# Astropianist/LumFuncMCMC

Hardware: AMD Instinct MI355X
Metric: walker-lnprob evals/sec (10^6 sources, 256 walkers) (higher is better)
Workload: dtype f64; 1 GPU; free completeness, single Schechter: 1000000 synthetic sources, 256 walkers in all (256 per GPU), 2 half-ensemble calls of 128 theta rows per step; walkers_per_gpu=256, walkers_total=256, variant=free, parallelism=1 GPU

## Files before the change

lumfuncmcmc_amd/csrc/lf_free.h:

```cpp
#pragma once
#include "lf_tile.h"

namespace lf {


template <bool THROUGH = false>
__device__ __forceinline__ void reduce_store512(const double* __restrict__ red, int wlo, int whi, double* __restrict__ out,
                                                size_t stride, int w0, int chunk, int tid) {
    const int w = tid >> 6, lane = tid & 63;
    if (w >= wlo && w < whi) {
        const double* row = red + w * PB + lane;
        double s0 = (row[0] + row[64]) + (row[128] + row[192]);
        double s1 = (row[256] + row[320]) + (row[384] + row[448]);
        const double s = wave_sum_dpp(s0 + s1);
        if (lane == 63) {
            if (THROUGH) __hip_atomic_store(out + (size_t)(w0 + w) * stride + chunk, s, __ATOMIC_RELAXED, __HIP_MEMORY_SCOPE_AGENT);
            else out[(size_t)(w0 + w) * stride + chunk] = s;
        }
    }
}

struct FreeArgs {
    int B, ntiles;
    int nchA, nchB;
    int nslot;
    int tile_stride;
    int skip_grid;
    int* queues;
    double* partA;
    double* partB;
    const double* cells;
    const double* nodes8;
    const int* deal;
    const int* cc_len;
    const int* cc_field;
    int nchC;
    int fin_ranks;
    double* partC;
    const int* wstat;
    const double* theta;
    double* out;
    double* wrec_w;
    int* wmode_w;
    int* wstat_w;
    double* wbase_w;
    const double* gq_rec;
    const double* gq_omega;
    const int* gq_rows;
    int nbq;
    int poll;
    int* err;
};

template <int ST, bool CENSUS, bool FUSED, bool STEP, class LA>
__device__ __forceinline__ void lf_free_body(const KConst& kc, const SrcArrays& sa, const NodeArrays& na, const double* __restrict__ wrec_arg,
                                             const int* __restrict__ wmode_arg, const FreeArgs& fa, const LA& la, const StepArgs& sp,
                                             const AcceptArgs& ap, unsigned long long t_pre = 0) {
    const double* wrec = FUSED ? fa.wrec_w : wrec_arg;
    const int* wmode = FUSED ? fa.wmode_w : wmode_arg;
    __shared__ MathTables tab;
    __shared__ TermTables tt;
    __shared__ __attribute__((aligned(16))) double red[PTW * PB];
    __shared__ __attribute__((aligned(16))) double wfc[PTW * MAXF * 8];
    __shared__ __attribute__((aligned(16))) double wsc[PTW * 8];
    __shared__ int sitem[2];
    __shared__ int sdeal[DEAL_MAX];
    __shared__ int scell;
    __shared__ int snosrc;
    const int tid = threadIdx.x;
    __shared__ int sstat[PTW];
    __shared__ double sbase[PTW];
    __shared__ double wlf[PTW * MAXF];
    __shared__ double sprop[PTW * 16];
    __shared__ double szz[PTW];
    __shared__ double spre[PTW * 2];
    if (!FUSED) {
        for (int i = tid; i < 256; i += PB) {
            tab.logt[i] = *reinterpret_cast<const double2*>(LOG_TABLE + 2 * i);
            tab.expt[i] = EXP_TABLE[i];
        }
        load_term_tables<PB>(&tt);
        if (fa.deal && tid < DEAL_LIST + fa.nchC + fa.nbq) sdeal[tid] = fa.deal[tid];
    }
    bool tables_loaded = !FUSED;
    const int wave_base = __builtin_amdgcn_readfirstlane(tid & ~63);
    auto fresh_tid = [&]() -> int {
        int m = -1;
        asm volatile("" : "+s"(m));
        return wave_base + __builtin_amdgcn_mbcnt_hi(m, __builtin_amdgcn_mbcnt_lo(m, 0));
    };
    unsigned xcc;
    asm volatile("s_getreg_b32 %0, hwreg(HW_REG_XCC_ID)" : "=s"(xcc));
    const int myq = (int)(xcc & 7u);
#ifdef LF_STAMPS
    __shared__ unsigned long long s_targs;
    unsigned long long* stamp = kc.stamps ? kc.stamps + (size_t)blockIdx.x * 8 : nullptr;
    if (stamp && tid == 0) {
        stamp[0] = t_pre ? t_pre : __builtin_amdgcn_s_memtime();
        stamp[5] = __builtin_amdgcn_s_memrealtime();
        s_targs = __builtin_amdgcn_s_memtime();
    }
    int nitems_done = 0;
    unsigned long long t_first = 0, t_sw = 0, t_loop = 0, t_red = 0;
    unsigned long long t_prep = 0, t_cells = 0, t_grid = 0;
    __shared__ unsigned long long s_ttab;
    __shared__ unsigned long long s_tp0;
    __shared__ unsigned long long s_tprep[8];
#endif

#pragma unroll 1
    for (int tile = ((int)blockIdx.x >> 3) % la.ntiles; tile < la.ntiles; tile += la.tile_stride) {
        const int w0 = tile * PTW;
        const int nw = min(PTW, la.B - w0);
        __builtin_assume(nw >= 1 && nw <= PTW);
        int* __restrict__ q = fa.queues + tile * QSTRIDE;
        int fgroup, frank;
        tile_ranks(tile, la.ntiles, la.tile_stride, fgroup, frank);
        const bool finisher = FUSED && fa.poll && frank == tile_finisher(fa.fin_ranks, fgroup);
        bool no_src = false;
        auto grab = [&]() -> int {
            if (no_src) return -1;
            for (int d = 0; d < 8; ++d) {
                const int qq = (myq + d) & 7;
                const int lo = (int)(((long long)qq * fa.nchA) >> 3), hi = (int)(((long long)(qq + 1) * fa.nchA) >> 3);
                if (hi <= lo) continue;
                const int i = atomicAdd(q + 1 + qq, 1);
                if (i < hi - lo) return lo + i;
            }
            return -1;
        };
        int ticket = 0;
        auto take_ticket = [&]() {
            if (!no_src) ticket = atomicAdd(q + 1 + myq, 1);
        };
        auto redeem = [&]() -> int {
            if (no_src) return -1;
            const int lo = (int)(((long long)myq * fa.nchA) >> 3), hi = (int)(((long long)(myq + 1) * fa.nchA) >> 3);
            if (ticket < hi - lo) return lo + ticket;
            return grab();
        };
        if (tile != ((int)blockIdx.x >> 3) % la.ntiles) __syncthreads();
        const int u = fresh_tid();
        if (FUSED) {
            const int pw = (int)(blockIdx.x >> 8) & 1;
            const int up = u - 64 * pw;
            if (up >= 0 && up < 64) {
                prepare_lane<false, true, STEP, LF_FREE>(kc, sp, la.theta, la.B, nullptr, nullptr, nullptr, nullptr, nullptr, 1,
                                          w0 + (up >> 3), up & 7, up >> 3, reinterpret_cast<double(*)[16]>(red), wfc, wsc, sstat, sbase, wlf,
#ifdef LF_STAMPS
                                          s_tprep,
#else
                                          nullptr,
#endif
                                          sprop, szz);
#ifdef LF_STAMPS
                if (up == 0) s_tp0 = __builtin_amdgcn_s_memtime();
#endif
            } else if (!tables_loaded) {
                const int t7 = u < 64 * pw ? u : u - 64;
                double2 lt = *reinterpret_cast<const double2*>(LOG_TABLE + 2 * min(t7, 255));
                double et = EXP_TABLE[min(t7, 255)];
                const int ndeal = fa.deal ? DEAL_LIST + fa.nchC + fa.nbq : 0;
                int d0 = ndeal ? fa.deal[min(t7, ndeal - 1)] : 0, d1 = ndeal ? fa.deal[min(t7 + 256, ndeal - 1)] : 0;
                asm volatile("" : "+v"(lt.x), "+v"(lt.y), "+v"(et), "+v"(d0), "+v"(d1));
                load_term_tables<PB - 64>(&tt, t7);
                if (t7 < 256) {
                    tab.logt[t7] = lt;
                    tab.expt[t7] = et;
                    if (t7 < ndeal) sdeal[t7] = d0;
                    if (t7 + 256 < ndeal) sdeal[t7 + 256] = d1;
                }
#ifdef LF_STAMPS
                if (t7 == 0) s_ttab = __builtin_amdgcn_s_memtime();
#endif
            }
            accept_terms_ahead<STEP>(sp, ap, w0, nw, u, spre);
            tables_loaded = true;
            __syncthreads();
        }
        if (u < 64) {
            const int st = FUSED ? sstat[min(u, nw - 1)] : fa.wstat[w0 + min(u, nw - 1)];
            const bool on = fa.nchC > 0 && u < nw && (st & STAT_CELLS);
            const bool need = u < nw && !on && (st & STAT_PRIOR_OK) && !(st & STAT_NEGINF);
            const int m = (int)__ballot(on);
            const unsigned long long mneed = __ballot(need);
            if (u == 0) {
                scell = m;
                no_src = mneed == 0ull;
                snosrc = no_src ? 1 : 0;
                sitem[0] = grab();
            }
        }
        if (!FUSED && u < nw * MAXF) {
            const int w = u / MAXF, f = u - w * MAXF;
            double* d = wfc + u * 8;
            int* di = reinterpret_cast<int*>(d + 4);
            if (f < kc.nf) {
                const double* __restrict__ r = wrec + (size_t)(w0 + w) * REC;
                const int* __restrict__ km = wmode + ((size_t)(w0 + w) * MAXF + f) * WM;
                d[0] = r[R_ALPHAC];
                d[F_V] = r[RF(f, F_V)];
                d[F_CA] = r[RF(f, F_CA)];
                d[F_CY] = r[RF(f, F_CY)] - H_LO - 0.5 / H_INV;
                d[7] = r[RF(f, F_CY)] - H_LO;
#pragma unroll
                for (int i = 0; i < 5; ++i) di[i] = km[i];
            }
        }
        if (!FUSED && u >= PB - PTW * 8) {
            const int t = u - (PB - PTW * 8), w = t >> 3, j = t & 7;
            if (w < nw) wsc[t] = wrec[(size_t)(w0 + w) * REC + j];
        }
        __syncthreads();
#ifdef LF_STAMPS
        t_prep = __builtin_amdgcn_s_memtime();
#endif
        const int cellmask = __builtin_amdgcn_readfirstlane(scell);
        const bool keep_own = finisher && uni(snosrc);
        double* __restrict__ sown = red + PB;
        auto fetch = [&](int w, int fld) {
            const double2* __restrict__ p = reinterpret_cast<const double2*>(wfc + (w * MAXF + fld) * 8);
            const double2 a = p[0], b = p[1], c = p[3];
            if (FUSED) {
                const int* __restrict__ ki = reinterpret_cast<const int*>(wfc + (w * MAXF + fld) * 8 + 4);
                return WalkerK{a.x, b.x, b.y, c.y, uni(ki[M_MODE]), uni(ki[M_KLO]), uni(ki[M_KHI]), uni(ki[M_KNE]), uni(ki[M_KAC])};
            }
            const int* __restrict__ km = wmode + ((size_t)(w0 + w) * MAXF + fld) * WM;
            return WalkerK{a.x, b.x, b.y, c.y, km[M_MODE], km[M_KLO], km[M_KHI], km[M_KNE], km[M_KAC]};
        };

        {
            const int v = wave_base >> 6;
#pragma unroll 1
            for (int vr = frank; vr < VF; vr += fgroup) {
            double acc = 0.0;
            const bool dealt = fa.deal != nullptr;
            const int cfirst = (vr - VF / 2 + VF) % VF;
            const int cb = dealt ? DEAL_LIST + uni(sdeal[vr]) : cfirst;
            const int cn = dealt ? uni(sdeal[vr + 1]) - uni(sdeal[vr]) : (cfirst < fa.nchC ? (fa.nchC - cfirst + VF - 1) / VF : 0);
            auto chunk_at = [&](int i) { return dealt ? uni(sdeal[cb + i]) : cb + i * VF; };
            if (fa.nchC > 0 && v < nw && ((cellmask >> v) & 1) && cn > 0) {
                auto load_cells = [&](double (&d)[CELL_REC], int cc) {
                    const int lane = fresh_tid() & 63;
                    const double2* __restrict__ src = reinterpret_cast<const double2*>(fa.cells + ((size_t)cc * 64 + lane) * CELL_REC);
                    static_assert(CELL_REC % 2 == 0, "16-byte loads");
#pragma unroll
                    for (int k = 0; k < CELL_REC / 2; ++k) {
                        const double2 a = src[k];
                        d[2 * k] = a.x;
                        d[2 * k + 1] = a.y;
                    }
                };
                auto field_of = [&](int cc) {
                    int f = 0;
#pragma unroll
                    for (int k = 1; k < MAXF; ++k) f += cc >= kc.cc_fstart[k] ? 1 : 0;
                    return f;
                };
                double nx[CELL_REC];
                load_cells(nx, chunk_at(0));
#pragma unroll 1
                for (int ci = 0; ci < cn; ++ci) {
                    const int cc = chunk_at(ci);
                    double cd[CELL_REC];
#pragma unroll
                    for (int k = 0; k < CELL_REC; ++k) cd[k] = nx[k];
                    if (ci + 1 < cn) load_cells(nx, chunk_at(ci + 1));
                    const WalkerK p = fetch(v, field_of(cc));
                    asm volatile("; LF_BEGIN cell items=1");
                    acc += cell_sum(cd, p, &tt);
                    asm volatile("; LF_END cell");
                    if (CENSUS && kc.forms && (fresh_tid() & 63) == 0) atomicAdd(kc.forms + FORM_CELL, (unsigned long long)uni(fa.cc_len[cc]));
                }
            }
            if (fa.nchC > 0 && v < nw) {
                acc = wave_sum_dpp(acc);
                const int ln = fresh_tid() & 63;
                double* __restrict__ row = fa.partC + (size_t)(w0 + v) * fa.nslot;
                if (ln == 63) {
                    if (keep_own) sown[v * 128 + vr] = acc;
                    else pstore<FUSED>(row + vr, acc);
                }
            }
            }
        }
#ifdef LF_STAMPS
        t_cells = __builtin_amdgcn_s_memtime();
#endif
        if (fa.nbq > 0) {
            const int v = wave_base >> 6;
            const int nq = fa.nbq;
#pragma unroll 1
            for (int vr = frank; vr < VF; vr += fgroup) {
            double bsum = 0.0;
            const bool dealt = fa.deal != nullptr;
            const int qb = dealt ? DEAL_LIST + fa.nchC + uni(sdeal[DEAL_BINS + vr]) : vr;
            const int qn = dealt ? uni(sdeal[DEAL_BINS + vr + 1]) - uni(sdeal[DEAL_BINS + vr]) : (vr < nq ? (nq - vr + VF - 1) / VF : 0);
            auto bin_at = [&](int i) { return dealt ? uni(sdeal[qb + i]) : qb + i * VF; };
            if (v < nw && qn > 0) {
                const double* __restrict__ sc = wsc + v * 8;
                const int mode = __builtin_amdgcn_readfirstlane(*reinterpret_cast<const int*>(wfc + (v * MAXF) * 8 + 4));
                const double* __restrict__ r = wfc + v * MAXF * 8 - 8;
                double vmin = r[RF(0, F_V)];
                for (int f = 1; f < kc.nf; ++f) vmin = fmin(vmin, r[RF(f, F_V)]);
                vmin = uni(vmin);
                const double alphaC = uni(sc[R_ALPHAC]);
                auto mine = [&](int c) { return mode != MODE_SKIP && !(kc.grid_parts > 1 && c % kc.grid_parts != kc.grid_part); };
                struct QRec {
                    double x, a4, L, PGL;
                };
                auto load_rec = [&](int c) -> QRec {
                    const int lane = fresh_tid() & 63;
                    const double2* __restrict__ src = reinterpret_cast<const double2*>(fa.gq_rec + ((size_t)c * 64 + lane) * 4);
                    const double2 a = src[0], b = src[1];
                    return QRec{a.x, a.y, b.x, b.y};
                };
                double* __restrict__ Tl = red + v * 64;
                QRec nx = load_rec(bin_at(0));
#pragma unroll 1
                for (int qi = 0; qi < qn; ++qi) {
                    const int c = bin_at(qi);
                    const QRec nd = nx;
                    const int nr = uni(fa.gq_rows[4 * c + 1]), off = uni(fa.gq_rows[4 * c + 2]);
                    if (qi + 1 < qn) nx = load_rec(bin_at(qi + 1));
                    if (mine(c)) {
                        const int lane = fresh_tid() & 63;
                        const double* __restrict__ om = fa.gq_omega + off + lane;
                        double o[8];
#pragma unroll
                        for (int i = 0; i < 8; ++i) o[i] = i < nr ? om[i * 64] : 0.0;
                        asm volatile("; LF_BEGIN qT items=1");
                        Tl[lane] = fexp_c(fma(uni(sc[R_C1]), nd.L - uni(sc[R_LSTAR]), uni(sc[R_C0])) - nd.PGL * uni(sc[R_Q]), &tab);
                        asm volatile("; LF_END qT");
                        const double a4min = __hiloint2double(__builtin_amdgcn_readlane(__double2hiint(nd.a4), 63),
                                                              __builtin_amdgcn_readlane(__double2loint(nd.a4), 63));
                        const bool bright = kc.specialise && alphaC > 0.0 && a4min * vmin > 37.5;
                        if (CENSUS && kc.forms && lane == 0)
                            atomicAdd(kc.forms + (bright ? FORM_NODE_BRIGHT : FORM_NODE_GENERAL), (unsigned long long)(64 * kc.nf));
                        const double s = field_sum_nf(kc, r, alphaC, nd.x, nd.a4, &tab, bright);
                        __builtin_amdgcn_wave_barrier();
                        asm volatile("; LF_BEGIN qdot items=1");
                        double R = 0.0;
#pragma unroll 1
                        for (int k0 = 0; k0 < nr; k0 += 8) {
                            double on[8];
#pragma unroll
                            for (int i = 0; i < 8; ++i) on[i] = k0 + 8 + i < nr ? om[(k0 + 8 + i) * 64] : 0.0;
#pragma unroll
                            for (int i = 0; i < 8; ++i) R = fma(Tl[min(k0 + i, 63)], o[i], R);
#pragma unroll
                            for (int i = 0; i < 8; ++i) o[i] = on[i];
                        }
                        asm volatile("; LF_END qdot");
                        bsum = fma(R, s, bsum);
                        __builtin_amdgcn_wave_barrier();
                    }
                }
            }
            if (v < nw) {
                bsum = wave_sum_dpp(bsum);
                const int ln = fresh_tid() & 63;
                double* __restrict__ row = fa.partB + (size_t)(w0 + v) * fa.nslot;
                if (ln == 63) {
                    if (keep_own) sown[v * 128 + 64 + vr] = bsum;
                    else pstore<FUSED>(row + vr, bsum);
                }
            }
            }
        } else
        {
            const int v = wave_base >> 6;
            const int nch64 = fa.nchB;
#pragma unroll 1
            for (int vr = frank; vr < VF; vr += fgroup) {
            double bsum = 0.0;
            if (v < nw && vr < nch64) {
                const double* __restrict__ sc = wsc + v * 8;
                const int mode = __builtin_amdgcn_readfirstlane(*reinterpret_cast<const int*>(wfc + (v * MAXF) * 8 + 4));
                const double* __restrict__ r = wfc + v * MAXF * 8 - 8;
                double vmin = r[RF(0, F_V)];
                for (int f = 1; f < kc.nf; ++f) vmin = fmin(vmin, r[RF(f, F_V)]);
                vmin = uni(vmin);
                const double alphaC = uni(sc[R_ALPHAC]);
                auto mine = [&](int c) { return mode != MODE_SKIP && !(kc.grid_parts > 1 && c % kc.grid_parts != kc.grid_part); };
                struct Node {
                    double G, PG, W, a3, a4, a4min;
                };
                auto load_nodes = [&](int c) -> Node {
                    const int lane = fresh_tid() & 63;
                    const double2* __restrict__ src = reinterpret_cast<const double2*>(fa.nodes8 + ((size_t)c * 64 + lane) * 8);
                    const double2 a = src[0], b = src[1], d = src[2];
                    return Node{a.x, a.y, b.x, b.y, d.x, d.y};
                };
                Node nx = load_nodes(vr);
#pragma unroll 1
                for (int c = vr; c < nch64; c += VF) {
                    const Node nd = nx;
                    if (c + VF < nch64) nx = load_nodes(c + VF);
                    if (mine(c)) {
                        const double a4min = uni(nd.a4min);
                        const double T = fexp_c(fma(uni(sc[R_C1]), nd.G - uni(sc[R_LSTAR]), uni(sc[R_C0])) - nd.PG * uni(sc[R_Q]), &tab);
                        const bool bright = kc.specialise && alphaC > 0.0 && a4min * vmin > 37.5;
                        if (CENSUS && kc.forms && (fresh_tid() & 63) == 0)
                            atomicAdd(kc.forms + (bright ? FORM_NODE_BRIGHT : FORM_NODE_GENERAL),
                                      (unsigned long long)(min(64, na.nnodes - c * 64) * kc.nf));
                        const double s = field_sum_nf(kc, r, alphaC, nd.a3, nd.a4, &tab, bright);
                        bsum = fma(nd.W * T, s, bsum);
                    }
                }
            }
            if (nch64 > 0 && v < nw) {
                bsum = wave_sum_dpp(bsum);
                const int ln = fresh_tid() & 63;
                double* __restrict__ row = fa.partB + (size_t)(w0 + v) * fa.nslot;
                if (ln == 63) {
                    if (keep_own) sown[v * 128 + 64 + vr] = bsum;
                    else pstore<FUSED>(row + vr, bsum);
                }
            }
            }
        }
#ifdef LF_STAMPS
        t_grid = __builtin_amdgcn_s_memtime();
#endif
        int item = sitem[0];
#pragma unroll 1
        while (item >= 0) {
#ifdef LF_STAMPS
            const unsigned long long ta = __builtin_amdgcn_s_memtime();
            if (t_first == 0) t_first = ta;
            unsigned long long tb = ta, tc = ta;
#endif
            __syncthreads();
            int t = fresh_tid();
            {
                const int c = item;
                const int s0 = uni(sa.chunk_start[c]), n = uni(sa.chunk_len[c]), fld = uni(sa.chunk_field[c]);
                const int kfirst = uni(sa.chunk_keys[KEY_STRIDE * c]), klast = uni(sa.chunk_keys[KEY_STRIDE * c + 1]),
                          kamax = uni(sa.chunk_keys[KEY_STRIDE * c + 4 + (wave_base >> 6)]);
                double x[ST];
                if (t == 0) take_ticket();
                if (n == PB * ST) {
                    typedef double __attribute__((ext_vector_type(2), aligned(8))) double2_a8;
                    const double2_a8* __restrict__ src = reinterpret_cast<const double2_a8*>(sa.a1 + s0 + t * ST);
#pragma unroll
                    for (int k = 0; k < ST / 2; ++k) {
                        const double2_a8 a = src[k];
                        x[2 * k] = a.x;
                        x[2 * k + 1] = a.y;
                    }
                } else {
                    const double* __restrict__ src = sa.a1 + s0;
#pragma unroll
                    for (int k = 0; k < ST; ++k) x[k] = src[min(t * ST + k, n - 1)];
                }
                if (t == 0) {
                    asm volatile("" ::"v"(x[ST - 1]));
                    sitem[0] = redeem();
                }
#ifdef LF_STAMPS
                tb = __builtin_amdgcn_s_memtime();
#endif
                const int npad = ST - min(max(n - t * ST, 0), ST);
                const int nwave = min(max(n - wave_base * ST, 0), 64 * ST);
                int rest = 0;
                WalkerK pn = fetch(0, fld);
#pragma unroll 1
                for (int w = 0; w < nw; ++w) {
                    const WalkerK p = pn;
                    pn = fetch(min(w + 1, nw - 1), fld);
                    double acc = 0.0;
                    if ((cellmask >> w) & 1) {
                    } else if (p.mode < MODE_SKIP && p.mode != MODE_SLOW && kc.tables && kfirst >= p.klo && klast <= p.khi && p.kac <= kamax) {
                        TabCoef C;
                        if (kc.specialise && kfirst >= p.kne) {
                            asm volatile("; LF_BEGIN table_noexp items=%0" ::"n"(ST));
                            table_lookup<ST>(C, x, p, true, &tt);
                            acc = table_terms<ST, true>(C, x, npad);
// ... 72 lines not shown
                        }
                        if (CENSUS && kc.forms && (t & 63) == 0) atomicAdd(kc.forms + form, (unsigned long long)nwave);
                        red[w * PB + t] = acc;
                    }
                }
#ifdef LF_STAMPS
                tc = __builtin_amdgcn_s_memtime();
#endif
                __syncthreads();
                t = fresh_tid();
                reduce_store512<FUSED>(red, 0, nw, fa.partA, (size_t)fa.nchA, w0, c, t);
                item = sitem[0];
            }
#ifdef LF_STAMPS
            ++nitems_done;
            if (tb != ta) {
                t_sw += tb - ta;
                t_loop += tc - tb;
                t_red += __builtin_amdgcn_s_memtime() - tc;
            }
#endif
        }
        if (FUSED && fa.poll && uni(snosrc)) {
            if (finisher) {
                const int t = fresh_tid(), v = t >> 6, ln = t & 63;
                const int nB = fa.nchB > 0 ? fa.nslot : 0, nC = fa.nchC > 0 ? fa.nslot : 0;
                if (v < nw) {
                    const bool own = ln % fgroup == frank;
                    double pre[2] = {0.0, 0.0};
                    if (own && ln < fa.nslot) pre[0] = sown[v * 128 + ln], pre[1] = sown[v * 128 + 64 + ln];
                    poll_finish(fa.partB, fa.partC, w0 + v, fa.nslot, nB, nC, ln, fa.err, pre, own);
                    finalize_wave<true>(fa.partA, 0, fa.nchA, fa.partB, nB, nB, nC > 0 ? fa.partC : nullptr, nC, (int)STAT_CELLS,
                                        sstat - w0, sbase - w0, w0 + v, ln, ap, la.out, nullptr, nullptr, 0,
                                        STEP ? sprop + v * 16 : nullptr, STEP ? szz + v : nullptr, STEP ? spre + 2 * v : nullptr, pre);
                }
            }
        } else if (FUSED) {
            count_finish(q, sitem[1], fgroup, nw, [&] { const int t = fresh_tid(); return TileThread{t, t >> 6, t & 63}; },
                         [&](int v, int ln) {
                             const int nB = fa.nchB > 0 ? fa.nslot : 0, nC = fa.nchC > 0 ? fa.nslot : 0;
                             finalize_wave<true>(fa.partA, fa.nchA, fa.nchA, fa.partB, nB, nB, nC > 0 ? fa.partC : nullptr, nC, (int)STAT_CELLS,
                                                 sstat - w0, sbase - w0, w0 + v, ln, ap, la.out, nullptr, nullptr, 0,
                                                 STEP ? sprop + v * 16 : nullptr, STEP ? szz + v : nullptr, STEP ? spre + 2 * v : nullptr);
                             if (fa.poll) empty_slots(fa.partB, fa.partC, w0 + v, fa.nslot, nB, nC, ln);
                         });
        }
    }
#ifdef LF_STAMPS
    if (stamp && tid == 0) {
        stamp[1] = __builtin_amdgcn_s_memtime();
        const bool noitems = nitems_done == 0;
        stamp[2] = (unsigned long long)nitems_done;
        if (noitems) {
            stamp[3] = t_prep - stamp[0];
            stamp[4] = t_cells - stamp[0];
            stamp[7] = t_grid - stamp[0];
            unsigned long long pk = 0;
            pk = ((s_targs - stamp[0]) >> 4) & 0xfffull;
            for (int i = 0; i < 4; ++i) pk |= (((s_tprep[i] - stamp[0]) >> 4) & 0xfffull) << (12 * (i + 1));
            stamp[2] = pk;
        } else {
            stamp[3] = t_first ? t_first - stamp[0] : 0;
            stamp[4] = t_sw;
            stamp[7] = t_loop;
        }
        stamp[6] = __builtin_amdgcn_s_memrealtime();
        kc.stamps[(size_t)gridDim.x * 8 + blockIdx.x] =
            !noitems ? t_red : (((s_ttab - stamp[0]) << 32) | ((s_tp0 - stamp[0]) & 0xffffffffull));
    }
#endif
}

template <int ST, bool CENSUS, bool FUSED = false>
__global__ __launch_bounds__(PB, 4) void lf_free(KConst kc, SrcArrays sa, NodeArrays na, const double* __restrict__ wrec_arg,
                                                 const int* __restrict__ wmode_arg, FreeArgs fa) {
    static_assert(!FUSED, "the one-launch form is the block entry below");
#ifdef LF_STAMPS
    const unsigned long long t_pre = __builtin_amdgcn_s_memtime();
#else
    const unsigned long long t_pre = 0;
#endif
    warm_kernarg<sizeof(KConst) + sizeof(SrcArrays) + sizeof(NodeArrays) + 2 * 8 + sizeof(FreeArgs)>();
    lf_free_body<ST, CENSUS, FUSED, false>(kc, sa, na, wrec_arg, wmode_arg, fa, fa, StepArgs{}, AcceptArgs{}, t_pre);
}

struct FreeLaunch {
    const double* theta;
    double* out;
    int B, ntiles;
    int tile_stride;
};
static_assert(sizeof(FreeLaunch) <= 64 - 8, "the block's pointer and the launch's fields: one line of kernel arguments");
struct FreeBlock {
    KConst kc;
    SrcArrays sa;
    NodeArrays na;
    FreeArgs fa;
};

typedef const __attribute__((address_space(4))) FreeBlock* FreeBlockPtr;

template <int ST, bool CENSUS, bool FUSED>
__global__ __launch_bounds__(PB, 4) void lf_free(FreeBlockPtr __restrict__ blkc, FreeLaunch la) {
    static_assert(FUSED && !CENSUS, "the block entry is the one-launch form");
    const FreeBlock* __restrict__ blk = (const FreeBlock*)blkc;
#ifdef LF_STAMPS
    const unsigned long long t_pre = __builtin_amdgcn_s_memtime();
// ... 15 lines not shown
```

lumfuncmcmc_amd/csrc/lf_kernels.h:

```cpp
#pragma once
#include "lf_layout.h"
#include "lf_math.h"

namespace lf {

constexpr int REC = 8 + 8 * MAXF;
constexpr int WM = 8;
enum { MODE_FAST = 0, MODE_SLOW = 1, MODE_NEGINF = 2, MODE_SKIP = 3, MODE_SKIPSRC = 4 };
enum { STAT_PRIOR_OK = 1, STAT_NEGINF = 2, STAT_SLOW = 4,
       STAT_CELLS = 8 };
constexpr int CELL_M = 8;
constexpr int CELL_REC = CELL_M + 2;
constexpr double CELL_RHO_G = 1.5e-2, CELL_RHO_H = 3.0e-3;
constexpr double ZCELL_RHO = 1.0e-3, ZCELL_X1 = 6.0e-3, ZCELL_X2 = 1.0e-5;
constexpr int ZCELL_M = 6;
constexpr int ZCELL_REC = ZCELL_M + 2;

enum { R_LSTAR = 0, R_C0 = 1, R_C1 = 2, R_Q = 3, R_ALPHAC = 4 };
enum { F_LF = 0, F_V = 1, F_CA = 2, F_CY = 3 };
__host__ __device__ constexpr int RF(int f, int slot) { return 8 + 8 * f + slot; }
enum { M_MODE = 0, M_KLO = 1, M_KHI = 2, M_KNE = 3, M_KAC = 4 };
enum { FORM_GENERAL = 0, FORM_GENERAL_NOEXP = 1, FORM_TABLE = 2, FORM_TABLE_NOEXP = 3, FORM_CAREFUL = 4, FORM_SKIPPED = 5,
       FORM_NODE_GENERAL = 6, FORM_NODE_BRIGHT = 7, FORM_CELL = 8, FORM_COUNT = 9 };
enum { Z_AL = 0, Z_BL = 1, Z_CL = 2, Z_AP = 3, Z_BP = 4, Z_CP = 5, Z_C1 = 6 };
// ... 80 lines not shown
}
__device__ __forceinline__ double u53(unsigned int hi, unsigned int lo) {
    return (double)((((unsigned long long)hi << 32) | lo) >> 11) * 1.1102230246251565e-16;
}
__device__ __forceinline__ double stretch_z(double a, double u) {
#pragma clang fp contract(off)
    const double t = (a - 1.0) * u;
    const double g = t + 1.0;
    const double g2 = g * g;
    return g2 / a;
}
__device__ __forceinline__ double stretch_point(double xj, double xk, double z) {
#pragma clang fp contract(off)
    const double d = xj - xk;
    const double dz = d * z;
    return xj - dz;
}
__device__ __forceinline__ void sampler_draw(unsigned long long step, int half, int w, int stream,
                                             unsigned long long seed, unsigned int (&r)[4]) {
    philox4x32((unsigned int)step, (unsigned int)(step >> 32) ^ ((unsigned int)half << 31), (unsigned int)w,
               (unsigned int)stream, (unsigned int)seed, (unsigned int)(seed >> 32), r);
}

template <int CTRL>
__device__ __forceinline__ int dpp_mov(int v) {
    return __builtin_amdgcn_update_dpp(0, v, CTRL, 0xf, 0xf, true);
}
template <int CTRL>
__device__ __forceinline__ double dpp_mov(double v) {
    return __hiloint2double(dpp_mov<CTRL>(__double2hiint(v)), dpp_mov<CTRL>(__double2loint(v)));
}
__device__ __forceinline__ double group8_sum(double v) {
    v += dpp_mov<0xB1>(v);
    v += dpp_mov<0x4E>(v);
    v += dpp_mov<0x141>(v);
    return v;
}
__device__ __forceinline__ int group8_or(int v) {
    v |= dpp_mov<0xB1>(v);
    v |= dpp_mov<0x4E>(v);
    v |= dpp_mov<0x141>(v);
    return v;
}

__device__ __forceinline__ int key_ceil(double v) {
    if (!(v == v)) return KEY_MAX;
    return (int)fmin(fmax(ceil(v), 0.0), (double)KEY_MAX);
}
__device__ __forceinline__ int key_floor(double v) {
    if (!(v == v)) return -1;
    return (int)fmin(fmax(floor(v), -1.0), (double)(KEY_MAX - 1));
}

template <bool BLOCK_SYNC, bool TOLDS = false, bool STEP = BLOCK_SYNC, int VAR = -1>
__device__ __forceinline__ void prepare_lane(const KConst& kc, const StepArgs& sp, const double* __restrict__ theta, int B,
                                             double* __restrict__ wrec, int* __restrict__ wstat,
                                             int* __restrict__ wmode, double* __restrict__ wbase, int* __restrict__ slow_list,
                                             int nqueue, int wq, int f, int grp, double (*sth)[16],
                                             double* __restrict__ l_fc = nullptr, double* __restrict__ l_sc = nullptr,
                                             int* __restrict__ l_stat = nullptr, double* __restrict__ l_base = nullptr,
                                             double* __restrict__ l_lf = nullptr, unsigned long long* tst = nullptr,
                                             double* __restrict__ l_prop = nullptr, double* __restrict__ l_zz = nullptr) {
#ifdef LF_STAMPS
#define LF_TST(i) do { if (tst && wq % 8 == 0 && f == 0) tst[i] = __builtin_amdgcn_s_memtime(); } while (0)
#else
#define LF_TST(i) do { } while (0)
#endif
    LF_TST(0);
    const int variant = VAR >= 0 ? VAR : kc.variant;
    const bool live = wq < B;
    const int w = live ? wq : B - 1;
    const bool has_f = f < kc.nf;
    struct {
        double pmax, lum_min, lum_max, a_min, u_min, u_max, lnom0, slc, sp, som, flim0, z_lo, z_hi, sz, sz2;
        int nsrc, kf_first, kf_last;
    } kf;
    struct {
        double lims[5][2], pivots[3], sch_al0, alpha0, fc_ratio, key_x0, zcell_rho;
    } pc;
    {
        int vz = 0;
        asm volatile("" : "+v"(vz));
        const double* __restrict__ lp = &kc.lims[0][0];
        const bool zv = variant == LF_ZEVOL;
#pragma unroll
        for (int i = 0; i < 10; ++i) pc.lims[i >> 1][i & 1] = zv && (i >> 1) >= LF_LIM_FLIM ? 0.0 : lp[i + vz];
        static_assert(LF_LIM_LSTAR < LF_LIM_FLIM && LF_LIM_PHISTAR < LF_LIM_FLIM && LF_LIM_SCH_AL < LF_LIM_FLIM && LF_LIM_ALPHA >= LF_LIM_FLIM,
                      "the z-evolving variant's limits come first");
#pragma unroll
        for (int i = 0; i < 3; ++i) pc.pivots[i] = zv ? (&kc.pivots[0])[i + vz] : 0.0;
        pc.sch_al0 = (&kc.sch_al0)[vz];
        pc.alpha0 = zv ? 0.0 : (&kc.alpha0)[vz];
        pc.fc_ratio = zv ? 0.0 : (&kc.fc_ratio)[vz];
        pc.key_x0 = zv ? 0.0 : (&kc.key_x0)[vz];
        pc.zcell_rho = zv ? (&kc.zcell_rho)[vz] : 0.0;
    }
    const bool stepping = STEP && sp.enabled;
    double t0 = 0.0, t1 = 0.0;
    if (!stepping) {
        const double* __restrict__ row = theta + (size_t)w * kc.ndim;
        t0 = row[min(f, kc.ndim - 1)];
        t1 = row[min(f + 8, kc.ndim - 1)];
    }
    kf.lum_min = kc.lum_min[f]; kf.lum_max = kc.lum_max[f]; kf.a_min = kc.a_min[f]; kf.slc = kc.slc[f]; kf.som = kc.som[f];
    kf.nsrc = kc.nsrc[f];
    if (variant == LF_ZEVOL) {
        kf.z_lo = kc.z_lo[f]; kf.z_hi = kc.z_hi[f]; kf.sz = kc.sz[f]; kf.sz2 = kc.sz2[f];
        kf.pmax = kf.u_min = kf.u_max = kf.lnom0 = kf.sp = kf.flim0 = 0.0; kf.kf_first = kf.kf_last = 0;
        asm volatile("" : "+v"(t0), "+v"(t1), "+v"(kf.lum_min), "+v"(kf.lum_max), "+v"(kf.a_min), "+v"(kf.slc), "+v"(kf.som), "+v"(kf.nsrc),
                          "+v"(kf.z_lo), "+v"(kf.z_hi), "+v"(kf.sz), "+v"(kf.sz2));
    } else {
        kf.pmax = kc.pmax[f]; kf.u_min = kc.u_min[f]; kf.u_max = kc.u_max[f]; kf.lnom0 = kc.lnom0_src[f]; kf.sp = kc.sp[f];
        kf.flim0 = kc.flim0[f]; kf.kf_first = kc.kf_first[f]; kf.kf_last = kc.kf_last[f];
        kf.z_lo = kf.z_hi = kf.sz = kf.sz2 = 0.0;
        asm volatile("" : "+v"(t0), "+v"(t1), "+v"(kf.lum_min), "+v"(kf.lum_max), "+v"(kf.a_min), "+v"(kf.slc), "+v"(kf.som), "+v"(kf.nsrc),
// ... 49 lines not shown
            const double n = (double)kf.nsrc;
            const double sph = aP * kf.sz2 + bP * kf.sz + n * cP;
            const double sls = aL * kf.sz2 + bL * kf.sz + n * (cL - LF_LREF);
            base = kf.som + n * LF_LNLN10 + LF_LN10 * sph + c1 * (kf.slc - sls);
        }
        if (live && f == 0) {
            double* d = TOLDS ? l_sc + grp * 8 : r;
            d[Z_AL] = aL; d[Z_BL] = bL; d[Z_CL] = cL;
            d[Z_AP] = aP; d[Z_BP] = bP; d[Z_CP] = cP;
            d[Z_C1] = c1;
        }
        if (live && has_f) {
            const double s0 = fabs(fma(2.0 * aL, kf.z_lo, bL)), s1 = fabs(fma(2.0 * aL, kf.z_hi, bL));
            (TOLDS ? l_fc + (grp * MAXF + f) * 8 : r + RF(f, 0))[0] = LF_LN10 * (fmax(s0, s1) + fabs(aL) * (1.0 / 128.0));
            cell_ok = kf.nsrc == 0 || (LF_LN10 * fmax(s0, s1) * pc.zcell_rho <= ZCELL_X1 &&
                                          LF_LN10 * fabs(aL) * pc.zcell_rho * pc.zcell_rho <= ZCELL_X2);
        }
        if (has_f && kf.nsrc > 0) {
            double lsmn, lsmx, phmn, phmx;
            quad_range(aL, bL, cL, kf.z_lo, kf.z_hi, lsmn, lsmx);
            quad_range(aP, bP, cP, kf.z_lo, kf.z_hi, phmn, phmx);
            const double tmax = kf.lum_max - lsmn, tmin = kf.lum_min - lsmx;
            const double vb = tmax < 2.9 ? (double)(__builtin_amdgcn_exp2f((float)tmax * 3.3219285f) * 1.0001f) + 1.0e-30 : 1.0e300;
            const double lb = LF_LNLN10 + LF_LN10 * phmn + fmin(c1 * tmin, c1 * tmax) - vb;
            m = (vb < 700.0 && lb > SAFE && lb + kf.a_min > SAFE) ? MODE_FAST : MODE_SLOW;
        }
    } else {
        const double Lstar = th[0], phistar = th[1];
        int k = 2;
        const double al = kc.fix_sch_al ? pc.sch_al0 : th[k++];
        const double alphaC = variant == LF_FREE ? th[k + kc.nf] : pc.alpha0;
        ok = ok && (Lstar >= pc.lims[LF_LIM_LSTAR][0]) && (Lstar <= pc.lims[LF_LIM_LSTAR][1]);
        ok = ok && (phistar >= pc.lims[LF_LIM_PHISTAR][0]) && (phistar <= pc.lims[LF_LIM_PHISTAR][1]);
        ok = ok && (al >= pc.lims[LF_LIM_SCH_AL][0]) && (al <= pc.lims[LF_LIM_SCH_AL][1]);
        ok = ok && (alphaC >= pc.lims[LF_LIM_ALPHA][0]) && (alphaC <= pc.lims[LF_LIM_ALPHA][1]);
        const double c0 = LF_LNLN10 + LF_LN10 * phistar, c1 = LF_LN10 * (al + 1.0);
        const double Q = exp10(LF_LREF - Lstar);
        asm volatile("" : "+v"(const_cast<double&>(Q)));
        LF_TST(2);
        if (has_f && kf.nsrc > 0) {
            const double n = (double)kf.nsrc;
            const double c0f = c0 + (variant == LF_FREE ? kf.lnom0 : 0.0);
            base = n * c0f + c1 * (kf.slc - n * (Lstar - LF_LREF)) - Q * kf.sp +
                   (variant == LF_FIXCOMP ? kf.som : 0.0);
        }
        if (live && f == 0) {
            double* d = TOLDS ? l_sc + grp * 8 : r;
            d[R_LSTAR] = Lstar;
            d[R_C0] = c0;
            d[R_C1] = c1;
            d[R_Q] = Q;
            d[R_ALPHAC] = alphaC;
        }
        if (has_f) {
            const double Flim = variant == LF_FREE ? th[k + f] : kf.flim0;
            ok = ok && (Flim >= pc.lims[LF_LIM_FLIM][0]) && (Flim <= pc.lims[LF_LIM_FLIM][1]);
            double lF = 0.0, V = 0.0;
            if (variant == LF_FREE) {
                const double b = -sqrt(pc.fc_ratio / (alphaC * alphaC));
                lF = log10(1.0e-17 * Flim);
                V = 1.0 / (Flim * exp10(b));
                const double cA = -alphaC * lF, cY = -(lF + b);
                int klo = KEY_MAX, khi = -1, kne = KEY_MAX, kac = KEY_MAX;
                if (nqueue > 0 && alphaC > 0.0 && alphaC < 1.0e4) {
                    const double xlo = fmax((G_NUM_LO + 2.0 * G_MARGIN - cA) / alphaC, H_LO + 2.0 * H_MARGIN - cY);
                    const double xhi = (G_NUM_HI - 2.0 * G_MARGIN - cA) / alphaC;
                    const double xne = 1.5740312677277188 - cY;
                    klo = key_ceil((xlo - pc.key_x0) * KEY_SCALE);
                    khi = key_floor((xhi - pc.key_x0) * KEY_SCALE);
                    kne = key_ceil((xne - pc.key_x0) * KEY_SCALE);
                    kac = key_ceil(alphaC * KEY_ASCALE);
                }
                cell_ok = kf.nsrc == 0 || (klo <= kf.kf_first && kf.kf_last <= khi);
                if (live && TOLDS) {
                    double* d = l_fc + (grp * MAXF + f) * 8;
                    int* di = reinterpret_cast<int*>(d + 4);
                    d[0] = alphaC;
                    d[F_V] = V;
                    d[F_CA] = cA;
                    d[F_CY] = cY - H_LO - 0.5 / H_INV;
                    d[7] = cY - H_LO;
                    di[M_KLO] = klo;
                    di[M_KHI] = khi;
                    di[M_KNE] = kne;
                    di[M_KAC] = kac;
                    l_lf[grp * MAXF + f] = lF;
                } else if (live) {
                    r[RF(f, F_LF)] = lF;
                    r[RF(f, F_V)] = V;
                    r[RF(f, F_CA)] = cA;
                    r[RF(f, F_CY)] = cY;
                    int* km = wmode + ((size_t)w * MAXF + f) * WM;
                    km[M_KLO] = klo;
                    km[M_KHI] = khi;
                    km[M_KNE] = kne;
                    km[M_KAC] = kac;
                }
            }
            LF_TST(3);
            if (kf.nsrc > 0) {
                const double vmax = kf.pmax * Q;
                const double tlo = kf.lum_min - Lstar, thi = kf.lum_max - Lstar;
                const double lbT = c0 + fmin(c1 * tlo, c1 * thi) - vmax;
                if (vmax > LF_UNDERFLOW) {
                    m = MODE_NEGINF;
                    neginf = 1;
                } else if (variant == LF_FREE) {
                    const double num = alphaC * (kf.a_min - lF);
                    const float an = (float)fmax(-num, 0.0);
                    const float lnfc_lo = num >= 0.0 ? -0.6932f
                                                     : -2.00002f * 0.69314724f * __builtin_amdgcn_logf(2.0f * (1.0f + an) * 1.000001f) - 0.01f;
                    const float x = (float)(kf.u_min * V) * 0.999999f;
                    const double lnOm = kf.lnom0 + (double)(lnfc_lo * (1.0f + 1.000001f / x));
                    m = (lbT > SAFE && lnOm > SAFE && lbT + lnOm > SAFE && kf.u_max * V < 1.0e6) ? MODE_FAST : MODE_SLOW;
                } else {
                    m = (lbT > SAFE && lbT + kf.a_min > SAFE) ? MODE_FAST : MODE_SLOW;
                }
            }
        }
    }
    LF_TST(4);
    base = group8_sum(base);
    const int bad = group8_or(ok ? 0 : 1);
    neginf = group8_or(neginf);
    if (bad) m = MODE_SKIP;
    else if (neginf) m = MODE_SKIPSRC;
    const int slow = group8_or(has_f && m == MODE_SLOW ? 1 : 0);
    const int nocell = group8_or(has_f && !(cell_ok && (m == MODE_FAST || kf.nsrc == 0)) ? 1 : 0);
    const int cells = kc.cells && (variant == LF_FREE ? nqueue > 0 : variant == LF_ZEVOL) && !bad && !neginf && !nocell;
    if (live && has_f) {
        if (TOLDS) reinterpret_cast<int*>(l_fc + (grp * MAXF + f) * 8 + 4)[M_MODE] = m;
        else wmode[((size_t)w * MAXF + f) * WM + M_MODE] = m;
    }
    if (live && f == 0) {
        const int st = (bad ? 0 : STAT_PRIOR_OK) | (neginf ? STAT_NEGINF : 0) | (slow ? STAT_SLOW : 0) | (cells ? STAT_CELLS : 0);
        if (TOLDS) {
            l_base[grp] = base;
            l_stat[grp] = st;
        } else {
            wbase[w] = base;
            wstat[w] = st;
            if (slow && slow_list) slow_list[1 + atomicAdd(slow_list, 1)] = w;
        }
    }
}

__global__ __launch_bounds__(64) void lf_prepare(KConst kc, StepArgs sp, const double* __restrict__ theta, int B,
                                                 double* __restrict__ wrec, int* __restrict__ wstat,
                                                 int* __restrict__ wmode, double* __restrict__ wbase, int* __restrict__ slow_list,
                                                 int* __restrict__ queue, int nqueue) {
    warm_kernarg<sizeof(KConst) + sizeof(StepArgs) + 7 * 8 + 8>();
    __shared__ double sth[8][16];
// ... 976 lines not shown
```

Baseline: 10.70 million walker-lnprob evals/s.

## Overlap walker preparation with bin sums via early barrier hook

Adds a barrier hook inside prepare_lane so the preparing wave publishes a per-walker out-of-bounds flag and joins the block barrier early, before the slow mode classification. The other waves then start the B-piece (bin sums) using that box flag instead of the full mode, while the preparing wave finishes. Cell sums are moved after the B-piece and the item grab follows a second barrier. This reorders the cross-wave schedule to hide preparation latency, at the cost of an extra barrier and more complex mode handling.

New measurement: 10.71 million walker-lnprob evals/s, median of 2. About the same (+0.1%).

```diff
diff --git a/lumfuncmcmc_amd/csrc/lf_free.h b/lumfuncmcmc_amd/csrc/lf_free.h
--- a/lumfuncmcmc_amd/csrc/lf_free.h
+++ b/lumfuncmcmc_amd/csrc/lf_free.h
@@ -19,6 +19,17 @@
         }
     }
 }
+
+struct BarrierA {
+    static constexpr bool empty = false;
+    unsigned long long* ta;
+    __device__ __forceinline__ void operator()() const {
+        __syncthreads();
+#ifdef LF_STAMPS
+        *ta = __builtin_amdgcn_s_memtime();
+#endif
+    }
+};
 
 struct FreeArgs {
     int B, ntiles;
@@ -74,6 +85,7 @@
     __shared__ double sprop[PTW * 16];
     __shared__ double szz[PTW];
     __shared__ double spre[PTW * 2];
+    __shared__ int sbox[PTW];
     if (!FUSED) {
         for (int i = tid; i < 256; i += PB) {
             tab.logt[i] = *reinterpret_cast<const double2*>(LOG_TABLE + 2 * i);
@@ -102,6 +114,7 @@
     }
     int nitems_done = 0;
     unsigned long long t_first = 0, t_sw = 0, t_loop = 0, t_red = 0;
+    unsigned long long t_a = 0, t_pb = 0;
     unsigned long long t_prep = 0, t_cells = 0, t_grid = 0;
     __shared__ unsigned long long s_ttab;
     __shared__ unsigned long long s_tp0;
@@ -144,19 +157,34 @@
         if (FUSED) {
             const int pw = (int)(blockIdx.x >> 8) & 1;
             const int up = u - 64 * pw;
-            if (up >= 0 && up < 64) {
-                prepare_lane<false, true, STEP, LF_FREE>(kc, sp, la.theta, la.B, nullptr, nullptr, nullptr, nullptr, nullptr, 1,
+            if ((wave_base >> 6) == pw) {
+#ifdef LF_STAMPS
+                unsigned long long* const tap = &t_a;
+#else
+                unsigned long long* const tap = nullptr;
+#endif
+                prepare_lane<false, true, STEP, LF_FREE, BarrierA>(kc, sp, la.theta, la.B, nullptr, nullptr, nullptr, nullptr, nullptr, 1,
                                           w0 + (up >> 3), up & 7, up >> 3, reinterpret_cast<double(*)[16]>(red), wfc, wsc, sstat, sbase, wlf,
 #ifdef LF_STAMPS
                                           s_tprep,
 #else
                                           nullptr,
 #endif
-                                          sprop, szz);
+                                          sprop, szz, sbox, BarrierA{tap});
 #ifdef LF_STAMPS
                 if (up == 0) s_tp0 = __builtin_amdgcn_s_memtime();
 #endif
-            } else if (!tables_loaded) {
+                const int st = sstat[min(up, nw - 1)];
+                const bool on = fa.nchC > 0 && up < nw && (st & STAT_CELLS);
+                const bool need = up < nw && !on && (st & STAT_PRIOR_OK) && !(st & STAT_NEGINF);
+                const int m = (int)__ballot(on);
+                const unsigned long long mneed = __ballot(need);
+                if (up == 0) {
+                    scell = m;
+                    snosrc = mneed == 0ull ? 1 : 0;
+                }
+            } else {
+              if (!tables_loaded) {
                 const int t7 = u < 64 * pw ? u : u - 64;
                 double2 lt = *reinterpret_cast<const double2*>(LOG_TABLE + 2 * min(t7, 255));
                 double et = EXP_TABLE[min(t7, 255)];
@@ -173,12 +201,16 @@
 #ifdef LF_STAMPS
                 if (t7 == 0) s_ttab = __builtin_amdgcn_s_memtime();
 #endif
-            }
-            accept_terms_ahead<STEP>(sp, ap, w0, nw, u, spre);
+              }
+              accept_terms_ahead<STEP>(sp, ap, w0, nw, u, spre);
+              __syncthreads();
+#ifdef LF_STAMPS
+              t_a = __builtin_amdgcn_s_memtime();
+#endif
+            }
             tables_loaded = true;
-            __syncthreads();
-        }
-        if (u < 64) {
+        }
+        if (!FUSED && u < 64) {
             const int st = FUSED ? sstat[min(u, nw - 1)] : fa.wstat[w0 + min(u, nw - 1)];
             const bool on = fa.nchC > 0 && u < nw && (st & STAT_CELLS);
             const bool need = u < nw && !on && (st & STAT_PRIOR_OK) && !(st & STAT_NEGINF);
@@ -211,95 +243,25 @@
             const int t = u - (PB - PTW * 8), w = t >> 3, j = t & 7;
             if (w < nw) wsc[t] = wrec[(size_t)(w0 + w) * REC + j];
         }
-        __syncthreads();
-#ifdef LF_STAMPS
-        t_prep = __builtin_amdgcn_s_memtime();
-#endif
-        const int cellmask = __builtin_amdgcn_readfirstlane(scell);
-        const bool keep_own = finisher && uni(snosrc);
+        const bool dealt = fa.deal != nullptr;
+        const auto fetch_mode0 = [&](int v) {
+            if (FUSED) return __builtin_amdgcn_readfirstlane(sbox[v]) ? (int)MODE_SKIP : (int)MODE_FAST;
+            return __builtin_amdgcn_readfirstlane(*reinterpret_cast<const int*>(wfc + (v * MAXF) * 8 + 4));
+        };
         double* __restrict__ sown = red + PB;
-        auto fetch = [&](int w, int fld) {
-            const double2* __restrict__ p = reinterpret_cast<const double2*>(wfc + (w * MAXF + fld) * 8);
-            const double2 a = p[0], b = p[1], c = p[3];
-            if (FUSED) {
-                const int* __restrict__ ki = reinterpret_cast<const int*>(wfc + (w * MAXF + fld) * 8 + 4);
-                return WalkerK{a.x, b.x, b.y, c.y, uni(ki[M_MODE]), uni(ki[M_KLO]), uni(ki[M_KHI]), uni(ki[M_KNE]), uni(ki[M_KAC])};
-            }
-            const int* __restrict__ km = wmode + ((size_t)(w0 + w) * MAXF + fld) * WM;
-            return WalkerK{a.x, b.x, b.y, c.y, km[M_MODE], km[M_KLO], km[M_KHI], km[M_KNE], km[M_KAC]};
-        };
-
-        {
-            const int v = wave_base >> 6;
-#pragma unroll 1
-            for (int vr = frank; vr < VF; vr += fgroup) {
-            double acc = 0.0;
-            const bool dealt = fa.deal != nullptr;
-            const int cfirst = (vr - VF / 2 + VF) % VF;
-            const int cb = dealt ? DEAL_LIST + uni(sdeal[vr]) : cfirst;
-            const int cn = dealt ? uni(sdeal[vr + 1]) - uni(sdeal[vr]) : (cfirst < fa.nchC ? (fa.nchC - cfirst + VF - 1) / VF : 0);
-            auto chunk_at = [&](int i) { return dealt ? uni(sdeal[cb + i]) : cb + i * VF; };
-            if (fa.nchC > 0 && v < nw && ((cellmask >> v) & 1) && cn > 0) {
-                auto load_cells = [&](double (&d)[CELL_REC], int cc) {
-                    const int lane = fresh_tid() & 63;
-                    const double2* __restrict__ src = reinterpret_cast<const double2*>(fa.cells + ((size_t)cc * 64 + lane) * CELL_REC);
-                    static_assert(CELL_REC % 2 == 0, "16-byte loads");
-#pragma unroll
-                    for (int k = 0; k < CELL_REC / 2; ++k) {
-                        const double2 a = src[k];
-                        d[2 * k] = a.x;
-                        d[2 * k + 1] = a.y;
-                    }
-                };
-                auto field_of = [&](int cc) {
-                    int f = 0;
-#pragma unroll
-                    for (int k = 1; k < MAXF; ++k) f += cc >= kc.cc_fstart[k] ? 1 : 0;
-                    return f;
-                };
-                double nx[CELL_REC];
-                load_cells(nx, chunk_at(0));
-#pragma unroll 1
-                for (int ci = 0; ci < cn; ++ci) {
-                    const int cc = chunk_at(ci);
-                    double cd[CELL_REC];
-#pragma unroll
-                    for (int k = 0; k < CELL_REC; ++k) cd[k] = nx[k];
-                    if (ci + 1 < cn) load_cells(nx, chunk_at(ci + 1));
-                    const WalkerK p = fetch(v, field_of(cc));
-                    asm volatile("; LF_BEGIN cell items=1");
-                    acc += cell_sum(cd, p, &tt);
-                    asm volatile("; LF_END cell");
-                    if (CENSUS && kc.forms && (fresh_tid() & 63) == 0) atomicAdd(kc.forms + FORM_CELL, (unsigned long long)uni(fa.cc_len[cc]));
-                }
-            }
-            if (fa.nchC > 0 && v < nw) {
-                acc = wave_sum_dpp(acc);
-                const int ln = fresh_tid() & 63;
-                double* __restrict__ row = fa.partC + (size_t)(w0 + v) * fa.nslot;
-                if (ln == 63) {
-                    if (keep_own) sown[v * 128 + vr] = acc;
-                    else pstore<FUSED>(row + vr, acc);
-                }
-            }
-            }
-        }
-#ifdef LF_STAMPS
-        t_cells = __builtin_amdgcn_s_memtime();
-#endif
+        auto piece_b = [&](const bool own) {
         if (fa.nbq > 0) {
             const int v = wave_base >> 6;
             const int nq = fa.nbq;
 #pragma unroll 1
             for (int vr = frank; vr < VF; vr += fgroup) {
             double bsum = 0.0;
-            const bool dealt = fa.deal != nullptr;
             const int qb = dealt ? DEAL_LIST + fa.nchC + uni(sdeal[DEAL_BINS + vr]) : vr;
             const int qn = dealt ? uni(sdeal[DEAL_BINS + vr + 1]) - uni(sdeal[DEAL_BINS + vr]) : (vr < nq ? (nq - vr + VF - 1) / VF : 0);
             auto bin_at = [&](int i) { return dealt ? uni(sdeal[qb + i]) : qb + i * VF; };
             if (v < nw && qn > 0) {
                 const double* __restrict__ sc = wsc + v * 8;
-                const int mode = __builtin_amdgcn_readfirstlane(*reinterpret_cast<const int*>(wfc + (v * MAXF) * 8 + 4));
+                const int mode = fetch_mode0(v);
                 const double* __restrict__ r = wfc + v * MAXF * 8 - 8;
                 double vmin = r[RF(0, F_V)];
                 for (int f = 1; f < kc.nf; ++f) vmin = fmin(vmin, r[RF(f, F_V)]);
@@ -362,7 +324,7 @@
                 const int ln = fresh_tid() & 63;
                 double* __restrict__ row = fa.partB + (size_t)(w0 + v) * fa.nslot;
                 if (ln == 63) {
-                    if (keep_own) sown[v * 128 + 64 + vr] = bsum;
+                    if (own) sown[v * 128 + 64 + vr] = bsum;
                     else pstore<FUSED>(row + vr, bsum);
                 }
             }
@@ -376,7 +338,7 @@
             double bsum = 0.0;
             if (v < nw && vr < nch64) {
                 const double* __restrict__ sc = wsc + v * 8;
-                const int mode = __builtin_amdgcn_readfirstlane(*reinterpret_cast<const int*>(wfc + (v * MAXF) * 8 + 4));
+                const int mode = fetch_mode0(v);
                 const double* __restrict__ r = wfc + v * MAXF * 8 - 8;
                 double vmin = r[RF(0, F_V)];
                 for (int f = 1; f < kc.nf; ++f) vmin = fmin(vmin, r[RF(f, F_V)]);
@@ -414,16 +376,111 @@
                 const int ln = fresh_tid() & 63;
                 double* __restrict__ row = fa.partB + (size_t)(w0 + v) * fa.nslot;
                 if (ln == 63) {
-                    if (keep_own) sown[v * 128 + 64 + vr] = bsum;
+                    if (own) sown[v * 128 + 64 + vr] = bsum;
                     else pstore<FUSED>(row + vr, bsum);
                 }
             }
             }
         }
+        };
+        if (FUSED) {
+            piece_b(finisher);
+#ifdef LF_STAMPS
+            t_pb = __builtin_amdgcn_s_memtime();
+#endif
+            __syncthreads();
+            no_src = uni(snosrc) != 0;
+            if (!no_src) {
+                if (finisher) {
+                    const int t = fresh_tid(), v = t >> 6;
+                    if (v < nw && (fa.nbq > 0 || fa.nchB > 0) && (t & 63) == 63) {
+                        double* __restrict__ row = fa.partB + (size_t)(w0 + v) * fa.nslot;
+                        for (int vr = frank; vr < VF; vr += fgroup) pstore<true>(row + vr, sown[v * 128 + 64 + vr]);
+                    }
+                }
+                if (u == 0) sitem[0] = grab();
+                __syncthreads();
+            }
+        } else
+        __syncthreads();
+#ifdef LF_STAMPS
+        t_prep = __builtin_amdgcn_s_memtime();
+#endif
+        const int cellmask = __builtin_amdgcn_readfirstlane(scell);
+        const bool keep_own = finisher && uni(snosrc);
+        auto fetch = [&](int w, int fld) {
+            const double2* __restrict__ p = reinterpret_cast<const double2*>(wfc + (w * MAXF + fld) * 8);
+            const double2 a = p[0], b = p[1], c = p[3];
+            if (FUSED) {
+                const int* __restrict__ ki = reinterpret_cast<const int*>(wfc + (w * MAXF + fld) * 8 + 4);
+                return WalkerK{a.x, b.x, b.y, c.y, uni(ki[M_MODE]), uni(ki[M_KLO]), uni(ki[M_KHI]), uni(ki[M_KNE]), uni(ki[M_KAC])};
+            }
+            const int* __restrict__ km = wmode + ((size_t)(w0 + w) * MAXF + fld) * WM;
+            return WalkerK{a.x, b.x, b.y, c.y, km[M_MODE], km[M_KLO], km[M_KHI], km[M_KNE], km[M_KAC]};
+        };
+
+        {
+            const int v = wave_base >> 6;
+#pragma unroll 1
+            for (int vr = frank; vr < VF; vr += fgroup) {
+            double acc = 0.0;
+            const int cfirst = (vr - VF / 2 + VF) % VF;
+            const int cb = dealt ? DEAL_LIST + uni(sdeal[vr]) : cfirst;
+            const int cn = dealt ? uni(sdeal[vr + 1]) - uni(sdeal[vr]) : (cfirst < fa.nchC ? (fa.nchC - cfirst + VF - 1) / VF : 0);
+            auto chunk_at = [&](int i) { return dealt ? uni(sdeal[cb + i]) : cb + i * VF; };
+            if (fa.nchC > 0 && v < nw && ((cellmask >> v) & 1) && cn > 0) {
+                auto load_cells = [&](double (&d)[CELL_REC], int cc) {
+                    const int lane = fresh_tid() & 63;
+                    const double2* __restrict__ src = reinterpret_cast<const double2*>(fa.cells + ((size_t)cc * 64 + lane) * CELL_REC);
+                    static_assert(CELL_REC % 2 == 0, "16-byte loads");
+#pragma unroll
+                    for (int k = 0; k < CELL_REC / 2; ++k) {
+                        const double2 a = src[k];
+                        d[2 * k] = a.x;
+                        d[2 * k + 1] = a.y;
+                    }
+                };
+                auto field_of = [&](int cc) {
+                    int f = 0;
+#pragma unroll
+                    for (int k = 1; k < MAXF; ++k) f += cc >= kc.cc_fstart[k] ? 1 : 0;
+                    return f;
+                };
+                double nx[CELL_REC];
+                load_cells(nx, chunk_at(0));
+#pragma unroll 1
+                for (int ci = 0; ci < cn; ++ci) {
+                    const int cc = chunk_at(ci);
+                    double cd[CELL_REC];
+#pragma unroll
+                    for (int k = 0; k < CELL_REC; ++k) cd[k] = nx[k];
+                    if (ci + 1 < cn) load_cells(nx, chunk_at(ci + 1));
+                    const WalkerK p = fetch(v, field_of(cc));
+                    asm volatile("; LF_BEGIN cell items=1");
+                    acc += cell_sum(cd, p, &tt);
+                    asm volatile("; LF_END cell");
+                    if (CENSUS && kc.forms && (fresh_tid() & 63) == 0) atomicAdd(kc.forms + FORM_CELL, (unsigned long long)uni(fa.cc_len[cc]));
+                }
+            }
+            if (fa.nchC > 0 && v < nw) {
+                acc = wave_sum_dpp(acc);
+                const int ln = fresh_tid() & 63;
+                double* __restrict__ row = fa.partC + (size_t)(w0 + v) * fa.nslot;
+                if (ln == 63) {
+                    if (keep_own) sown[v * 128 + vr] = acc;
+                    else pstore<FUSED>(row + vr, acc);
+                }
+            }
+            }
+        }
+#ifdef LF_STAMPS
+        t_cells = __builtin_amdgcn_s_memtime();
+#endif
+        if (!FUSED) piece_b(false);
 #ifdef LF_STAMPS
         t_grid = __builtin_amdgcn_s_memtime();
 #endif
-        int item = sitem[0];
+        int item = FUSED && no_src ? -1 : sitem[0];
 #pragma unroll 1
         while (item >= 0) {
 #ifdef LF_STAMPS
@@ -602,7 +659,7 @@
         const bool noitems = nitems_done == 0;
         stamp[2] = (unsigned long long)nitems_done;
         if (noitems) {
-            stamp[3] = t_prep - stamp[0];
+            stamp[3] = (t_prep - stamp[0]) | (FUSED ? (((t_a - stamp[0]) & 0xfffffull) << 20) | (((t_pb - stamp[0]) & 0xfffffull) << 40) : 0ull);
             stamp[4] = t_cells - stamp[0];
             stamp[7] = t_grid - stamp[0];
             unsigned long long pk = 0;
diff --git a/lumfuncmcmc_amd/csrc/lf_kernels.h b/lumfuncmcmc_amd/csrc/lf_kernels.h
--- a/lumfuncmcmc_amd/csrc/lf_kernels.h
+++ b/lumfuncmcmc_amd/csrc/lf_kernels.h
@@ -156,7 +156,11 @@
     return (int)fmin(fmax(floor(v), -1.0), (double)(KEY_MAX - 1));
 }
 
-template <bool BLOCK_SYNC, bool TOLDS = false, bool STEP = BLOCK_SYNC, int VAR = -1>
+struct NoHook {
+    static constexpr bool empty = true;
+    __device__ __forceinline__ void operator()() const {}
+};
+template <bool BLOCK_SYNC, bool TOLDS = false, bool STEP = BLOCK_SYNC, int VAR = -1, class HOOK = NoHook>
 __device__ __forceinline__ void prepare_lane(const KConst& kc, const StepArgs& sp, const double* __restrict__ theta, int B,
                                              double* __restrict__ wrec, int* __restrict__ wstat,
                                              int* __restrict__ wmode, double* __restrict__ wbase, int* __restrict__ slow_list,
@@ -164,7 +168,9 @@
                                              double* __restrict__ l_fc = nullptr, double* __restrict__ l_sc = nullptr,
                                              int* __restrict__ l_stat = nullptr, double* __restrict__ l_base = nullptr,
                                              double* __restrict__ l_lf = nullptr, unsigned long long* tst = nullptr,
-                                             double* __restrict__ l_prop = nullptr, double* __restrict__ l_zz = nullptr) {
+                                             double* __restrict__ l_prop = nullptr, double* __restrict__ l_zz = nullptr,
+                                             int* __restrict__ l_box = nullptr, HOOK hook = HOOK{}) {
+    static_assert(HOOK::empty || (TOLDS && VAR == LF_FREE), "the hook sits on the FREE variant's path to LDS");
 #ifdef LF_STAMPS
 #define LF_TST(i) do { if (tst && wq % 8 == 0 && f == 0) tst[i] = __builtin_amdgcn_s_memtime(); } while (0)
 #else
@@ -320,10 +326,10 @@
             d[R_Q] = Q;
             d[R_ALPHAC] = alphaC;
         }
+        double lF = 0.0, V = 0.0;
         if (has_f) {
             const double Flim = variant == LF_FREE ? th[k + f] : kf.flim0;
             ok = ok && (Flim >= pc.lims[LF_LIM_FLIM][0]) && (Flim <= pc.lims[LF_LIM_FLIM][1]);
-            double lF = 0.0, V = 0.0;
             if (variant == LF_FREE) {
                 const double b = -sqrt(pc.fc_ratio / (alphaC * alphaC));
                 lF = log10(1.0e-17 * Flim);
@@ -366,6 +372,13 @@
                 }
             }
             LF_TST(3);
+        }
+        if (!HOOK::empty) {
+            const int box = group8_or(ok ? 0 : 1);
+            if (live && f == 0) l_box[grp] = box;
+            hook();
+        }
+        if (has_f) {
             if (kf.nsrc > 0) {
                 const double vmax = kf.pmax * Q;
                 const double tlo = kf.lum_min - Lstar, thi = kf.lum_max - Lstar;
```
